# kdavila/lecturemath

Measured on AMD Instinct MI355X. Metric: frames/sec end-to-end binarize+CC+group @1080p, higher is better.
Workload: dtype u8

## Files before the change

lecturemath_amd/csrc/lm_group.hip:

```cpp
#include "lm_stream.h"

#include <sched.h>

#include <algorithm>
#include <atomic>
#include <chrono>
#include <thread>
#include <unordered_map>
#include <vector>

#define LM_SJ_TILE 256

__global__ void __launch_bounds__(256) lm_k_selfjoin(const unsigned long long* __restrict__ box, int n, int* __restrict__ n_pairs,
                                                     int2* __restrict__ pairs, int cap_pairs)
{
    __shared__ unsigned long long s_box[LM_SJ_TILE];
    __shared__ int s_base;
    unsigned mine = 0, off = 0;
    for (int pass = 0; pass < 2; pass++) {
        for (int rt = blockIdx.y * LM_SJ_TILE; rt < n; rt += gridDim.y * LM_SJ_TILE) {
            const int tile = (n - rt < LM_SJ_TILE) ? n - rt : LM_SJ_TILE;
            __syncthreads();
            if ((int)threadIdx.x < tile) s_box[threadIdx.x] = box[rt + threadIdx.x];
            __syncthreads();
// ... 116 lines not shown
{
    const int X0 = it.x0 + un.tx * LM_GT, Y0 = it.y0 + un.ty * LM_GT;
    const int wx0 = r.min_x >> 5, nw = (r.max_x >> 5) - wx0 + 1;
    const int ya = r.min_y > Y0 ? r.min_y : Y0, yb = r.max_y < Y0 + LM_GT - 1 ? r.max_y : Y0 + LM_GT - 1;
    const int ja = (X0 >> 5) > wx0 ? (X0 >> 5) - wx0 : 0;
    const int jb = ((X0 + LM_GT - 1) >> 5) - wx0 < nw - 1 ? ((X0 + LM_GT - 1) >> 5) - wx0 : nw - 1;
    const int tw = jb - ja + 1, total = (tw > 0 && yb >= ya) ? tw * (yb - ya + 1) : 0;
    bool hit = false;
    for (int idx = threadIdx.x; idx < total && !hit; idx += blockDim.x) {
        const int rr = idx / tw, j = ja + (idx - rr * tw);
        unsigned wbits = crop[r.crop_off + (unsigned long long)((ya + rr - r.min_y) * nw + j)];
        const int xw = (wx0 + j) * 32;
        if (xw < X0) wbits &= (X0 - xw >= 32) ? 0u : (0xffffffffu << (X0 - xw));
        if (xw + 31 >= X0 + LM_GT) wbits &= (xw >= X0 + LM_GT) ? 0u : (0xffffffffu >> (xw + 32 - (X0 + LM_GT)));
        hit = wbits != 0u;
    }
    if (hit) *s_hit = 1;
}

LM_DEV void lm_gimg_single_write(const LmGimgItem& it, const LmGimgUnit& un, const LmCcRec& r, const uint32_t* __restrict__ crop, uint32_t* __restrict__ bits)
{
    const int X0 = it.x0 + un.tx * LM_GT, Y0 = it.y0 + un.ty * LM_GT;
    const int wx0 = r.min_x >> 5, nw = (r.max_x >> 5) - wx0 + 1;
    const int tw = (it.w - un.tx * LM_GT < LM_GT) ? it.w - un.tx * LM_GT : LM_GT;
    const int th = (it.h - un.ty * LM_GT < LM_GT) ? it.h - un.ty * LM_GT : LM_GT;
    const int bw = (it.w + 31) >> 5;
    for (int t = threadIdx.x; t < 2 * LM_GT; t += blockDim.x) {
        const int yy = t >> 1, k = t & 1, y = Y0 + yy;
        if (yy >= th || un.tx * 2 + k >= bw || y < r.min_y || y > r.max_y) continue;
        const int xa = X0 + 32 * k;
        const int c0 = (xa >> 5) - wx0, sh = xa & 31;
        const uint32_t* row = crop + r.crop_off + (unsigned long long)(y - r.min_y) * nw;
        const unsigned lo = (c0 >= 0 && c0 < nw) ? row[c0] : 0u;
        const unsigned hi = (sh && c0 + 1 >= 0 && c0 + 1 < nw) ? row[c0 + 1] : 0u;
        unsigned w = sh ? ((lo >> sh) | (hi << (32 - sh))) : lo;
        const int valid = tw - 32 * k;
        if (valid < 32) w &= valid <= 0 ? 0u : ((1u << valid) - 1u);
        if (w) bits[it.bits_off + (long long)(un.ty * LM_GT + yy) * bw + un.tx * 2 + k] = w;
    }
}

LM_DEV int lm_gimg_vmin(int item_max, double thr)
{
    const double mx = (double)item_max;
    int vmin = (int)(thr * mx);
    if (vmin < 0) vmin = 0;
    while (vmin > 0 && (double)(vmin - 1) / mx >= thr) vmin--;
    while ((double)vmin / mx < thr) vmin++;
    return vmin;
}

LM_DEV bool lm_gimg_single_tile(const LmGimgItem& it) { return it.w <= LM_GT && it.h <= LM_GT; }

__global__ void __launch_bounds__(256) lm_k_gimg_max(const LmGimgItem* __restrict__ items, const LmGimgUnit* __restrict__ units,
                                                     const unsigned* __restrict__ n_units_p, const LmGimgMember* __restrict__ members,
                                                     const LmCcRec* __restrict__ cc, const uint32_t* __restrict__ crop,
                                                     int32_t* __restrict__ item_max, double thr, uint32_t* __restrict__ bits)
{
    __shared__ int s_mask[LM_GT * LM_GT];
    __shared__ int s_max;
    const int n_units = (int)*n_units_p;
    for (int u = blockIdx.x; u < n_units; u += gridDim.x) {
        const LmGimgUnit un = units[u];
        const LmGimgItem it = items[un.item];
        if (threadIdx.x == 0) s_max = 0;
        if (un.mem_cnt == 1 && thr > 0.0) {
            const LmGimgMember mem = members[un.mem_off];
            const LmCcRec r = cc[mem.cc];
            __syncthreads();
            lm_gimg_single_hit(it, un, r, crop, &s_max);
            __syncthreads();
            const int tile_max = s_max ? mem.count : 0;
            if (threadIdx.x == 0 && tile_max) atomicMax(&item_max[un.item], tile_max);
            if (lm_gimg_single_tile(it) && tile_max && tile_max >= lm_gimg_vmin(tile_max, thr)) lm_gimg_single_write(it, un, r, crop, bits);
            __syncthreads();
            continue;
        }
        lm_gimg_accumulate(it, un, members, cc, crop, s_mask);
        int mx = 0;
        for (int i = threadIdx.x; i < LM_GT * LM_GT; i += blockDim.x) mx = s_mask[i] > mx ? s_mask[i] : mx;
        if (mx) atomicMax(&s_max, mx);
        __syncthreads();
        const int tile_max = s_max;
        if (threadIdx.x == 0 && tile_max) atomicMax(&item_max[un.item], tile_max);
        if (lm_gimg_single_tile(it) && tile_max) lm_gimg_write_tile(it, un, s_mask, tile_max, thr, bits);
        __syncthreads();
    }
}

__global__ void __launch_bounds__(256) lm_k_gimg_write(const LmGimgItem* __restrict__ items, const LmGimgUnit* __restrict__ units,
                                                       const unsigned* __restrict__ n_units_p, const LmGimgMember* __restrict__ members,
                                                       const LmCcRec* __restrict__ cc, const uint32_t* __restrict__ crop,
                                                       const int32_t* __restrict__ item_max, double thr, uint32_t* __restrict__ bits)
{
    __shared__ int s_mask[LM_GT * LM_GT];
    const int n_units = (int)*n_units_p;
    for (int u = blockIdx.x; u < n_units; u += gridDim.x) {
        const LmGimgUnit un = units[u];
        const LmGimgItem it = items[un.item];
        if (lm_gimg_single_tile(it) && item_max[un.item] > 0) continue;
        if (un.mem_cnt == 1 && thr > 0.0 && item_max[un.item] > 0) {
            const LmGimgMember mem = members[un.mem_off];
            if (mem.count >= lm_gimg_vmin(item_max[un.item], thr)) lm_gimg_single_write(it, un, cc[mem.cc], crop, bits);
            continue;
        }
        lm_gimg_accumulate(it, un, members, cc, crop, s_mask);
        lm_gimg_write_tile(it, un, s_mask, item_max[un.item], thr, bits);
        __syncthreads();
    }
}

struct LmRenderItem { int32_t x0, y0, w, h; long long bits_off; };

#define LM_RT_ROWS 64
#define LM_RT_COLS 256
#define LM_RT_PITCH (LM_RT_COLS / 32 + 1)
#define LM_RT_PLANE (LM_RT_ROWS * LM_RT_PITCH)
#define LM_RT_MAXHIT 96
#define LM_RT_WPL 4

LM_DEV void lm_render_paint(const LmRenderItem& it, int X0, int Y0, const uint32_t* __restrict__ bits, unsigned* s_pl, int lane, int nl)
{
    const int xa = it.x0 > X0 ? it.x0 : X0, xb = (it.x0 + it.w < X0 + LM_RT_COLS) ? it.x0 + it.w : X0 + LM_RT_COLS;
    const int ya = it.y0 > Y0 ? it.y0 : Y0, yb = (it.y0 + it.h < Y0 + LM_RT_ROWS) ? it.y0 + it.h : Y0 + LM_RT_ROWS;
    const int bw = (it.w + 31) >> 5;
    const int jlo = (xa - X0) >> 5, nw = ((xb - 1 - X0) >> 5) - jlo + 1;
    const int total = nw * (yb - ya);
    const float inv = 1.0f / (float)nw;
    const uint32_t* src = bits + it.bits_off + (long long)(ya - it.y0) * bw;
    for (int idx0 = lane; idx0 < total; idx0 += nl * LM_RT_WPL) {
        unsigned lo[LM_RT_WPL], hi[LM_RT_WPL];
        int col[LM_RT_WPL], slot[LM_RT_WPL];
#pragma unroll
        for (int u = 0; u < LM_RT_WPL; u++) {
            const int idx = idx0 + u * nl;
            int yy = (int)((float)idx * inv);
            int j = idx - yy * nw;
            if (j < 0) { yy--; j += nw; }
            if (j >= nw) { yy++; j -= nw; }
            col[u] = X0 + 32 * (jlo + j);
            const int d = col[u] - it.x0;
            const int sw = d >> 5;
            const uint32_t* r = src + (long long)yy * bw;
            const bool on = idx < total;
            lo[u] = (on && sw >= 0 && sw < bw) ? r[sw] : 0u;
            hi[u] = (on && (d & 31) && sw + 1 < bw) ? r[sw + 1] : 0u;
            slot[u] = (ya - Y0 + yy) * LM_RT_PITCH + jlo + j;
        }
#pragma unroll
        for (int u = 0; u < LM_RT_WPL; u++) {
            const int sh = (col[u] - it.x0) & 31;
            unsigned c = sh ? ((lo[u] >> sh) | (hi[u] << (32 - sh))) : lo[u];
            if (col[u] < xa) c &= 0xffffffffu << (xa - col[u]);
            if (col[u] + 32 > xb) c &= 0xffffffffu >> (col[u] + 32 - xb);
            for (int p = 0; p < 8 && c; p++) c &= atomicXor(&s_pl[p * LM_RT_PLANE + slot[u]], c);
        }
    }
}

__global__ void __launch_bounds__(256) lm_k_render_items(const long long* __restrict__ frame_item_off, int F, const int32_t* __restrict__ gpf,
                                                         const int32_t* __restrict__ ages, const int32_t* __restrict__ ages_off,
                                                         const int32_t* __restrict__ bounds, const int64_t* __restrict__ gitem_first,
                                                         const int64_t* __restrict__ gbits_off, LmRenderItem* __restrict__ out)
{
    for (int f = blockIdx.x; f < F; f += gridDim.x)
    for (long long i = frame_item_off[f] + threadIdx.x; i < frame_item_off[f + 1]; i += blockDim.x) {
    const int gi = gpf[i];
    const int32_t* a = ages + ages_off[gi];
    const int na = ages_off[gi + 1] - ages_off[gi];
    LmRenderItem ri;
    ri.x0 = bounds[gi * 4 + 0]; ri.y0 = bounds[gi * 4 + 2];
    ri.w = bounds[gi * 4 + 1] - ri.x0 + 1; ri.h = bounds[gi * 4 + 3] - ri.y0 + 1;
    ri.bits_off = 0;
    if (na < 2) {
        ri.w = 0; ri.h = 0;
    } else {
        int lo = 0, hi = na - 1;
        while (hi - lo > 1) {
            const int mid = (lo + hi) >> 1;
            if (a[mid] < f) lo = mid; else hi = mid;
        }
        const int sidx = lo;
        ri.bits_off = gbits_off[gitem_first[gi] + sidx];
    }
    out[i] = ri;
    }
}

__global__ void __launch_bounds__(256) lm_k_render_frames(const long long* __restrict__ frame_item_off,
                                                          const LmRenderItem* __restrict__ items, const uint32_t* __restrict__ bits,
                                                          int first_frame, int W, int H, uint8_t* __restrict__ out)
{
    __shared__ unsigned s_pl[8 * LM_RT_PLANE];
    __shared__ LmRenderItem s_hit[LM_RT_MAXHIT];
    __shared__ unsigned s_pre[LM_RT_MAXHIT + 1];
    __shared__ int s_nhit;
    const int f = first_frame + blockIdx.z;
    const int X0 = blockIdx.x * LM_RT_COLS, Y0 = blockIdx.y * LM_RT_ROWS;
    for (int i = threadIdx.x; i < 8 * LM_RT_PLANE; i += blockDim.x) s_pl[i] = 0;
    if (threadIdx.x == 0) s_nhit = 0;
    __syncthreads();
    const long long i0 = frame_item_off[f], i1 = frame_item_off[f + 1];
#pragma unroll 2
    for (long long ib = i0 + threadIdx.x; ib < i1; ib += blockDim.x) {
        const LmRenderItem mine = items[ib];
        if (mine.x0 < X0 + LM_RT_COLS && mine.x0 + mine.w > X0 && mine.y0 < Y0 + LM_RT_ROWS && mine.y0 + mine.h > Y0) {
            const int slot = atomicAdd(&s_nhit, 1);
            if (slot < LM_RT_MAXHIT) s_hit[slot] = mine;
            else lm_render_paint(mine, X0, Y0, bits, s_pl, 0, 1);
        }
    }
    __syncthreads();
    const int nhit = s_nhit < LM_RT_MAXHIT ? s_nhit : LM_RT_MAXHIT;
    {
        const int lane = lm_lane();
        if (threadIdx.x < 64) {
            unsigned carry = 0;
            for (int h0 = 0; h0 < nhit; h0 += 64) {
                const int h = h0 + lane;
                unsigned words = 0;
                if (h < nhit) {
                    const LmRenderItem it = s_hit[h];
                    const int xa = it.x0 > X0 ? it.x0 : X0, xb = (it.x0 + it.w < X0 + LM_RT_COLS) ? it.x0 + it.w : X0 + LM_RT_COLS;
                    const int ya = it.y0 > Y0 ? it.y0 : Y0, yb = (it.y0 + it.h < Y0 + LM_RT_ROWS) ? it.y0 + it.h : Y0 + LM_RT_ROWS;
                    const int jlo = (xa - X0) >> 5, nw = ((xb - 1 - X0) >> 5) - jlo + 1;
                    words = (nw > 0 && yb > ya) ? (unsigned)(nw * (yb - ya)) : 0u;
                }
                const unsigned incl = lm_wave_incl_scan(words);
                if (h < nhit) s_pre[h] = carry + incl - words;
                carry += (unsigned)__shfl((int)incl, 63);
            }
            if (lane == 0) s_pre[nhit] = carry;
        }
    }
    __syncthreads();
    {
        const unsigned total = s_pre[nhit];
        for (unsigned g0 = threadIdx.x; g0 < total; g0 += blockDim.x * LM_RT_WPL) {
            unsigned lo[LM_RT_WPL], hi[LM_RT_WPL];
            int col[LM_RT_WPL], slot[LM_RT_WPL], xa_[LM_RT_WPL], xb_[LM_RT_WPL], x0_[LM_RT_WPL];
#pragma unroll
            for (int u = 0; u < LM_RT_WPL; u++) {
                const unsigned g = g0 + (unsigned)u * blockDim.x;
                lo[u] = 0; hi[u] = 0; col[u] = 0; slot[u] = 0; xa_[u] = 0; xb_[u] = 0; x0_[u] = 0;
                if (g < total) {
                    int a = 0, b2 = nhit;
                    while (b2 - a > 1) {
                        const int mid = (a + b2) >> 1;
                        if (s_pre[mid] <= g) a = mid; else b2 = mid;
                    }
                    const LmRenderItem it = s_hit[a];
                    const int xa = it.x0 > X0 ? it.x0 : X0, xb = (it.x0 + it.w < X0 + LM_RT_COLS) ? it.x0 + it.w : X0 + LM_RT_COLS;
                    const int ya = it.y0 > Y0 ? it.y0 : Y0;
                    const int bw = (it.w + 31) >> 5;
                    const int jlo = (xa - X0) >> 5, nw = ((xb - 1 - X0) >> 5) - jlo + 1;
                    const int idx = (int)(g - s_pre[a]);
                    int yy = (int)((float)idx * (1.0f / (float)nw));
                    int j = idx - yy * nw;
                    if (j < 0) { yy--; j += nw; }
                    if (j >= nw) { yy++; j -= nw; }
                    col[u] = X0 + 32 * (jlo + j);
                    const int d = col[u] - it.x0;
                    const int sw = d >> 5;
                    const uint32_t* r = bits + it.bits_off + (long long)(ya - it.y0 + yy) * bw;
                    lo[u] = (sw >= 0 && sw < bw) ? r[sw] : 0u;
                    hi[u] = ((d & 31) && sw + 1 < bw) ? r[sw + 1] : 0u;
                    slot[u] = (ya - Y0 + yy) * LM_RT_PITCH + jlo + j;
                    xa_[u] = xa; xb_[u] = xb; x0_[u] = it.x0;
                }
            }
#pragma unroll
            for (int u = 0; u < LM_RT_WPL; u++) {
                if (g0 + (unsigned)u * blockDim.x >= total) continue;
                const int sh = (col[u] - x0_[u]) & 31;
                unsigned c = sh ? ((lo[u] >> sh) | (hi[u] << (32 - sh))) : lo[u];
                if (col[u] < xa_[u]) c &= 0xffffffffu << (xa_[u] - col[u]);
                if (col[u] + 32 > xb_[u]) c &= 0xffffffffu >> (col[u] + 32 - xb_[u]);
                for (int p = 0; p < 8 && c; p++) c &= atomicXor(&s_pl[p * LM_RT_PLANE + slot[u]], c);
            }
        }
    }
    __syncthreads();
    uint8_t* dst = out + (long long)blockIdx.z * W * H;
    const bool vec = ((W & 15) == 0) && ((((uintptr_t)out) & 15) == 0);
    for (int i = threadIdx.x; i < LM_RT_ROWS * LM_RT_COLS / 16; i += blockDim.x) {
        const int yy = i / (LM_RT_COLS / 16), xq = i - yy * (LM_RT_COLS / 16);
        const int y = Y0 + yy, x = X0 + xq * 16;
        if (y >= H || x >= W) continue;
        unsigned pl[8], upper = 0;
#pragma unroll
        for (int p = 0; p < 8; p++) {
            pl[p] = (s_pl[p * LM_RT_PLANE + yy * LM_RT_PITCH + (xq >> 1)] >> (16 * (xq & 1))) & 0xffffu;
            if (p) upper |= pl[p];
        }
        unsigned o[4];
        if (!upper) {
#pragma unroll
            for (int q = 0; q < 4; q++) o[q] = ((((pl[0] >> (4 * q)) & 15u) * 0x00204081u) & 0x01010101u) * 0xffu;
        } else {
#pragma unroll
            for (int q = 0; q < 4; q++) {
                o[q] = 0;
                for (int t = 0; t < 4; t++) {
                    unsigned k = 0;
                    for (int p = 0; p < 8; p++) k |= ((pl[p] >> (4 * q + t)) & 1u) << p;
                    o[q] |= ((0u - k) & 0xffu) << (8 * t);
                }
            }
        }
        uint8_t* d = dst + (long long)y * W + x;
        if (vec) {
            *(uint4*)d = make_uint4(o[0], o[1], o[2], o[3]);
        } else {
            for (int k = 0; k < 16 && x + k < W; k++) d[k] = (uint8_t)(o[k >> 2] >> (8 * (k & 3)));
        }
    }
}

__global__ void __launch_bounds__(256) lm_k_frame_sums(const uint8_t* __restrict__ frames, long long px, unsigned long long* __restrict__ sums)
{
    const uint8_t* f = frames + (long long)blockIdx.y * px;
    const bool vec = ((((uintptr_t)f) & 15) == 0);
    unsigned long long acc = 0;
    const long long n16 = vec ? (px >> 4) : 0;
    for (long long i = (long long)blockIdx.x * blockDim.x + threadIdx.x; i < n16; i += (long long)gridDim.x * blockDim.x) {
        const uint4 v = *(const uint4*)(f + (i << 4));
        unsigned s4 = 0;
#if LM_HIP_EMULATED
        const unsigned w[4] = {v.x, v.y, v.z, v.w};
        for (int k = 0; k < 4; k++) s4 += (w[k] & 0xffu) + ((w[k] >> 8) & 0xffu) + ((w[k] >> 16) & 0xffu) + (w[k] >> 24);
#else
        s4 = __builtin_amdgcn_sad_u8(v.x, 0u, s4); s4 = __builtin_amdgcn_sad_u8(v.y, 0u, s4);
        s4 = __builtin_amdgcn_sad_u8(v.z, 0u, s4); s4 = __builtin_amdgcn_sad_u8(v.w, 0u, s4);
#endif
        acc += s4;
    }
    for (long long i = (n16 << 4) + (long long)blockIdx.x * blockDim.x + threadIdx.x; i < px; i += (long long)gridDim.x * blockDim.x) acc += f[i];
    __shared__ unsigned long long s_acc;
    if (threadIdx.x == 0) s_acc = 0;
    __syncthreads();
    const unsigned lo = lm_wave_sum((unsigned)(acc & 0xffffffu)), mid = lm_wave_sum((unsigned)((acc >> 24) & 0xffffffu));
    const unsigned hi = lm_wave_sum((unsigned)(acc >> 48));
    if (lm_lane() == 0) atomicAdd(&s_acc, (unsigned long long)lo + ((unsigned long long)mid << 24) + ((unsigned long long)hi << 48));
    __syncthreads();
    if (threadIdx.x == 0 && s_acc) atomicAdd(&sums[blockIdx.y], s_acc);
}

struct LmBitImage { int32_t x0, y0, w, h; long long src_off, bits_off; };

__global__ void __launch_bounds__(256) lm_k_img_pack(const LmBitImage* __restrict__ items, int n, const uint8_t* __restrict__ src,
                                                     uint32_t* __restrict__ bits)
{
    for (int it = blockIdx.y; it < n; it += gridDim.y) {
        const LmBitImage im = items[it];
        const int bw = (im.w + 31) >> 5;
        for (int i = blockIdx.x * blockDim.x + threadIdx.x; i < im.h * bw; i += gridDim.x * blockDim.x) {
            const int y = i / bw, k = i - y * bw;
            const uint8_t* p = src + im.src_off + (long long)y * im.w + k * 32;
            const int lim = (im.w - k * 32 < 32) ? im.w - k * 32 : 32;
            unsigned word = 0;
            for (int b = 0; b < lim; b++) word |= (unsigned)(p[b] != 0) << b;
            bits[im.bits_off + i] = word;
        }
    }
}
// ... 365 lines not shown
{
    for (int k = blockIdx.y; k < n_items; k += gridDim.y) {
        const LmGimgItem it = items[k];
        const int bw = (it.w + 31) >> 5;
        const long long px = (long long)it.w * it.h;
        for (long long i = (long long)blockIdx.x * blockDim.x + threadIdx.x; i < px; i += (long long)gridDim.x * blockDim.x) {
            const int y = (int)(i / it.w), x = (int)(i - (long long)y * it.w);
            images[it.img_off + i] = ((bits[it.bits_off + (long long)y * bw + (x >> 5)] >> (x & 31)) & 1u) ? 255 : 0;
        }
    }
}

struct LmGroups {
    LmStream* s;
    int max_gap, min_times, t_window;
    double min_recall, img_thr;
    int n_frames, n_uniq0;
    int64_t n_split;
    std::vector<int32_t> uniq_cc;
    std::vector<int64_t> ulist_off;
    std::vector<int32_t> ulist_cc;
    std::vector<int32_t> assign;
    std::vector<int32_t> stable;
    int64_t total_intersections;
    std::vector<int64_t> grp_off; std::vector<int32_t> grp_members;
    std::vector<int32_t> gid_of_unique;
    std::vector<int64_t> ages_off; std::vector<int32_t> ages;
    std::vector<int64_t> gpf_off; std::vector<int32_t> gpf;
    std::vector<int32_t> conf_g1, conf_g2; std::vector<int64_t> conf_matched, conf_unmatched, conf_union; std::vector<double> conf_inter;
    std::vector<int32_t> bounds;
    std::vector<int64_t> gimg_off;
    std::vector<int64_t> gimg_item_off;
    bool have_pairs = false, have_nbr = false;
    std::vector<int32_t> pair_a, pair_b, pair_match;
    std::vector<int64_t> tov_off; std::vector<int32_t> tov_other; std::vector<double> tov_recall, tov_precision;
    std::vector<int64_t> aov_off; std::vector<int32_t> aov_other, aov_matched, aov_size_other, aov_size_self;
    std::vector<uint8_t> gimg_host;
    int n_stable = 0;
    long long n_adj = 0, n_aov = 0, n_tov = 0;
    unsigned* d_adj_off = nullptr; int32_t *d_adj = nullptr, *d_arow = nullptr, *d_match = nullptr;
    unsigned *d_aov_off = nullptr, *d_tov_off = nullptr;
    int32_t *d_aov_j = nullptr, *d_aov_other = nullptr, *d_aov_matched = nullptr, *d_aov_size_other = nullptr, *d_aov_size_self = nullptr;
    int32_t* d_tov_other = nullptr; double *d_tov_recall = nullptr, *d_tov_precision = nullptr;
    LmGimgItem* d_items = nullptr;
    int n_items = 0;
    uint32_t* d_gbits = nullptr;
    std::vector<int64_t> gbits_off;
    long long* d_frame_item_off = nullptr;
    LmRenderItem* d_render_items = nullptr;
    std::vector<void*> d_owned;
    char* arena = nullptr;
    size_t arena_cap = 0, arena_used = 0, arena_want = 0;
    bool arena_cached = false;
    char* pin = nullptr;
    size_t pin_cap = 0, pin_used = 0;
    std::vector<void*> pin_owned;
    bool pin_cached = false;
    size_t pin_want = 0;
};

static void* lm_galloc(LmGroups* g, size_t bytes)
{
    const size_t need = (bytes + 255) & ~(size_t)255;
    g->arena_want += need;
    if (g->arena && g->arena_used + need <= g->arena_cap) {
        void* p = g->arena + g->arena_used;
        g->arena_used += need;
        return p;
    }
    void* p = nullptr;
    if (hipMalloc(&p, need ? need : 256) != hipSuccess) { lm_set_error("lm_group_run: hipMalloc(%zu) failed", need); return nullptr; }
    g->d_owned.push_back(p);
    return p;
}

static void* lm_gpin(LmGroups* g, size_t bytes)
{
    const size_t need = (bytes + 255) & ~(size_t)255;
    g->pin_want += need;
    if (g->pin && g->pin_used + need <= g->pin_cap) {
        void* p = g->pin + g->pin_used;
        g->pin_used += need;
        return p;
    }
    void* p = nullptr;
    if (hipHostMalloc(&p, need ? need : 256) != hipSuccess) { lm_set_error("lm_group_run: hipHostMalloc(%zu) failed", need); return nullptr; }
    g->pin_owned.push_back(p);
    return p;
}

#define LM_G_ARRAYS 40
enum {
    LM_G_UNIQ_CC = 0, LM_G_ULIST_OFF, LM_G_ULIST_CC, LM_G_ASSIGN, LM_G_STABLE, LM_G_PAIR_A, LM_G_PAIR_B, LM_G_PAIR_MATCH,
    LM_G_TOV_OFF, LM_G_TOV_OTHER, LM_G_TOV_RECALL, LM_G_TOV_PRECISION, LM_G_AOV_OFF, LM_G_AOV_OTHER, LM_G_AOV_MATCHED,
    LM_G_AOV_SIZE_OTHER, LM_G_AOV_SIZE_SELF, LM_G_GRP_OFF, LM_G_GRP_MEMBERS, LM_G_GID, LM_G_AGES_OFF, LM_G_AGES, LM_G_GPF_OFF,
    LM_G_GPF, LM_G_CONF_G1, LM_G_CONF_G2, LM_G_CONF_MATCHED, LM_G_CONF_UNMATCHED, LM_G_CONF_UNION, LM_G_CONF_INTER, LM_G_BOUNDS,
    LM_G_GIMG_OFF, LM_G_GIMG_ITEM_OFF, LM_G_GIMG, LM_G_SCALARS
};

template <class T> static int lm_upload(LmGroups* g, const std::vector<T>& v, T** d, hipStream_t st)
{
    *d = (T*)lm_galloc(g, (v.size() ? v.size() : 1) * sizeof(T));
    if (!*d) return LM_ERR_HIP;
    if (v.empty()) return LM_OK;
    void* stage = lm_gpin(g, v.size() * sizeof(T));
    if (!stage) return LM_ERR_HIP;
    memcpy(stage, v.data(), v.size() * sizeof(T));
    LM_HIP(hipMemcpyAsync(*d, stage, v.size() * sizeof(T), hipMemcpyHostToDevice, st));
    return LM_OK;
}

template <class T> static int lm_download(LmGroups* g, const T* d, size_t n, std::vector<T>& v, hipStream_t st)
// ... 486 lines not shown
            const unsigned long long b = s_box[(size_t)sidx_of_unique[u]];
            x0 = std::min(x0, (int)(b & 0xffff)); x1 = std::max(x1, (int)((b >> 16) & 0xffff));
            y0 = std::min(y0, (int)((b >> 32) & 0xffff)); y1 = std::max(y1, (int)(b >> 48));
            slot_group[(size_t)i] = gi;
            slot_cc[(size_t)i] = g->uniq_cc[u];
        }
        g->bounds[(size_t)gi * 4 + 0] = x0; g->bounds[(size_t)gi * 4 + 1] = x1; g->bounds[(size_t)gi * 4 + 2] = y0; g->bounds[(size_t)gi * 4 + 3] = y1;
        const int w = x1 - x0 + 1, h = y1 - y0 + 1;
        const int ns = (int)(g->ages_off[(size_t)gi + 1] - g->ages_off[gi]) - 1;
        const long long ntiles = (long long)((w + LM_GT - 1) / LM_GT) * ((h + LM_GT - 1) / LM_GT);
        for (int j = 0; j < ns; j++) {
            LmGimgItem it;
            it.x0 = x0; it.y0 = y0; it.w = w; it.h = h;
            it.img_off = g->gimg_off.back();
            it.bits_off = bit_words;
            g->gbits_off.push_back(bit_words);
            g->gimg_off.push_back(it.img_off + (int64_t)w * h);
            bit_words += (long long)h * ((w + 31) >> 5);
            tile_off.push_back(tile_off.back() + ntiles);
            items.push_back(it);
        }
        g->gimg_item_off.push_back((int64_t)items.size());
    }
    const int n_items = (int)items.size();
    const long long n_tiles = tile_off.back();
    g->n_items = n_items;
    tm.mark("  gimg: items (host)");
    g->d_gbits = (uint32_t*)lm_galloc(g, (size_t)std::max<long long>(bit_words, 1) * sizeof(uint32_t));
    if (!g->d_gbits) return LM_ERR_HIP;
    int64_t* d_gitem_first = nullptr;
    int32_t *d_ages = nullptr;
    if (n_items > 0) {
        LmGimgTab T;
        int32_t *d_slot_group, *d_slot_unique, *d_slot_cc, *d_ulist_frame, *d_bounds_g;
        int64_t *d_ages_off64, *d_ulist_off, *d_tile_off;
        std::vector<int64_t> gitem_first(g->gimg_item_off.begin(), g->gimg_item_off.end() - 1);
        if (lm_upload(g, slot_group, &d_slot_group, st) || lm_upload(g, g->grp_members, &d_slot_unique, st) || lm_upload(g, slot_cc, &d_slot_cc, st) ||
            lm_upload(g, g->ages, &d_ages, st) || lm_upload(g, g->ages_off, &d_ages_off64, st) || lm_upload(g, gitem_first, &d_gitem_first, st) ||
            lm_upload(g, g->ulist_off, &d_ulist_off, st) || lm_upload(g, ulist_frame, &d_ulist_frame, st) || lm_upload(g, tile_off, &d_tile_off, st) ||
            lm_upload(g, items, &g->d_items, st) || lm_upload(g, g->bounds, &d_bounds_g, st))
            return LM_ERR_HIP;
        T.slot_group = d_slot_group; T.slot_unique = d_slot_unique; T.slot_cc = d_slot_cc; T.n_slots = (int)g->grp_members.size();
        T.ages = d_ages; T.ages_off = d_ages_off64; T.gitem_first = d_gitem_first; T.ulist_off = d_ulist_off; T.ulist_frame = d_ulist_frame;
        T.tile_off = d_tile_off; T.bounds = d_bounds_g;
        const size_t nt1 = (size_t)std::max<long long>(n_tiles, 1);
        const int n_chunks = (int)((n_tiles + LM_SCAN_CHUNK - 1) / LM_SCAN_CHUNK);
        unsigned* d_tile_cnt = (unsigned*)lm_galloc(g, (nt1 + 1) * sizeof(unsigned));
        unsigned* d_tile_moff = (unsigned*)lm_galloc(g, (nt1 + 1) * sizeof(unsigned));
        unsigned* d_chunk = (unsigned*)lm_galloc(g, ((size_t)n_chunks + 2) * sizeof(unsigned));
        LmGimgUnit* d_units = (LmGimgUnit*)lm_galloc(g, nt1 * sizeof(LmGimgUnit));
        int32_t* d_max = (int32_t*)lm_galloc(g, (size_t)n_items * sizeof(int32_t));
        unsigned* d_nunits = (unsigned*)lm_galloc(g, 256);
        if (!d_tile_cnt || !d_tile_moff || !d_chunk || !d_units || !d_max || !d_nunits) return LM_ERR_HIP;
        LM_HIP(hipMemsetAsync(d_tile_cnt, 0, (nt1 + 1) * sizeof(unsigned), st));
        LM_HIP(hipMemsetAsync(d_nunits, 0, 256, st));
        LM_HIP(hipMemsetAsync(d_max, 0, (size_t)n_items * sizeof(int32_t), st));
        LM_HIP(hipMemsetAsync(g->d_gbits, 0, (size_t)std::max<long long>(bit_words, 1) * sizeof(uint32_t), st));
        const unsigned sb = lm_gblocks(T.n_slots, 4, 16384);
        hipLaunchKernelGGL((lm_k_gimg_members<0>), dim3(sb), dim3(256), 0, st, T, d_tile_cnt, (const unsigned*)nullptr, (LmGimgMember*)nullptr, s->cc);
        hipLaunchKernelGGL(lm_k_scan_chunks, dim3((unsigned)std::max(n_chunks, 1)), dim3(1024), 0, st, d_tile_cnt, d_tile_moff, n_tiles, d_chunk);
        hipLaunchKernelGGL(lm_k_scan_u32, dim3(1), dim3(1024), 0, st, d_chunk, d_chunk, n_chunks, d_tot + 5);
        hipLaunchKernelGGL(lm_k_scan_add, dim3(lm_gblocks(n_tiles + 1, 256, 4096)), dim3(256), 0, st, d_tile_moff, n_tiles, d_chunk, n_chunks);
        unsigned long long h_nmem = 0;
        LM_HIP(hipMemcpyAsync(&h_nmem, d_tot + 5, sizeof(h_nmem), hipMemcpyDeviceToHost, st));
        LM_HIP(hipStreamSynchronize(st));
        if (h_nmem >= (1ull << 32)) { lm_set_error("lm_group_run: %llu group-image tile members (limit 2^32)", h_nmem); return LM_ERR_CAPACITY; }
        LmGimgMember* d_members = (LmGimgMember*)lm_galloc(g, (size_t)std::max<unsigned long long>(h_nmem, 1) * sizeof(LmGimgMember));
        if (!d_members) return LM_ERR_HIP;
        LM_HIP(hipMemsetAsync(d_tile_cnt, 0, (nt1 + 1) * sizeof(unsigned), st));
        hipLaunchKernelGGL((lm_k_gimg_members<1>), dim3(sb), dim3(256), 0, st, T, d_tile_cnt, d_tile_moff, d_members, s->cc);
        hipLaunchKernelGGL(lm_k_gimg_units, dim3(lm_gblocks(n_tiles, 256, 4096)), dim3(256), 0, st, d_tile_moff, n_tiles, d_tile_off, g->d_items, n_items,
                           g->img_thr > 0.0 ? 0 : 1, d_units, d_nunits);
        tm.mark("  gimg: member + tile tables (device)", st, true);
        const unsigned nb = LM_HIP_EMULATED ? 2u : (unsigned)std::min<long long>(std::max<long long>(n_tiles, 1), 8192);
        hipLaunchKernelGGL(lm_k_gimg_max, dim3(nb), dim3(256), 0, st, g->d_items, d_units, d_nunits, d_members, s->cc, s->crop, d_max, g->img_thr, g->d_gbits);
        hipLaunchKernelGGL(lm_k_gimg_write, dim3(nb), dim3(256), 0, st, g->d_items, d_units, d_nunits, d_members, s->cc, s->crop, d_max, g->img_thr,
                           g->d_gbits);
        LM_HIP(hipGetLastError());
        if (tm.on) {
            unsigned nu_ = 0;
            (void)hipMemcpyAsync(&nu_, d_nunits, 4, hipMemcpyDeviceToHost, st);
            (void)hipStreamSynchronize(st);
            fprintf(stderr, "[lm_group]   groups %d items %d tile members %llu tiles %lld visited %u conflicts %zu\n", nG, n_items, h_nmem, n_tiles, nu_,
                    g->conf_g1.size());
        }
        tm.mark("  gimg: max + write", st, true);
    }
    if (reconstruct_tables) {
        std::vector<long long> fio(g->gpf_off.begin(), g->gpf_off.end());
        std::vector<int32_t> ages_off32(g->ages_off.begin(), g->ages_off.end());
        int32_t *d_gpf, *d_ages_off, *d_bounds;
        int64_t* d_gbits_off;
        const size_t n_ritems = g->gpf.size();
        g->d_render_items = (LmRenderItem*)lm_galloc(g, std::max<size_t>(n_ritems, 1) * sizeof(LmRenderItem));
        if (!g->d_render_items) return LM_ERR_HIP;
        if (lm_upload(g, fio, &g->d_frame_item_off, st)) return LM_ERR_HIP;
        if (n_ritems) {
            if (lm_upload(g, g->gpf, &d_gpf, st) || lm_upload(g, ages_off32, &d_ages_off, st) || lm_upload(g, g->bounds, &d_bounds, st) ||
                lm_upload(g, g->gbits_off, &d_gbits_off, st))
                return LM_ERR_HIP;
            hipLaunchKernelGGL(lm_k_render_items, dim3(lm_gblocks(F, 1, 16384)), dim3(256), 0, st, g->d_frame_item_off, F, d_gpf,
                               d_ages, d_ages_off, d_bounds, d_gitem_first, d_gbits_off, g->d_render_items);
        }
    }
    LM_HIP(hipGetLastError());
    LM_HIP(hipStreamSynchronize(st));
    tm.mark("render tables + final sync");
    return LM_OK;
}

static int lm_group_materialize_pairs(LmGroups* g)
{
    if (g->have_pairs) return LM_OK;
    std::vector<int32_t> adj, arow, match;
    hipStream_t st = nullptr;
    if (g->n_adj > 0 && (lm_download(g, g->d_adj, (size_t)g->n_adj, adj, st) || lm_download(g, g->d_arow, (size_t)g->n_adj, arow, st) ||
                         lm_download(g, g->d_match, (size_t)g->n_adj, match, st)))
        return LM_ERR_HIP;
    g->pair_a.clear(); g->pair_b.clear(); g->pair_match.clear();
    for (long long e = 0; e < g->n_adj; e++)
        if (arow[(size_t)e] < adj[(size_t)e]) {
            g->pair_a.push_back(g->stable[arow[(size_t)e]]); g->pair_b.push_back(g->stable[adj[(size_t)e]]); g->pair_match.push_back(match[(size_t)e]);
        }
    g->have_pairs = true;
    return LM_OK;
}

static int lm_group_materialize_neighbours(LmGroups* g)
{
    if (g->have_nbr) return LM_OK;
    hipStream_t st = nullptr;
    const size_t nU = g->uniq_cc.size();
    const int nS = g->n_stable;
    std::vector<unsigned> aoff, toff;
    g->tov_off.assign(nU + 1, 0); g->aov_off.assign(nU + 1, 0);
    if (nS > 0) {
        if (lm_download(g, g->d_aov_off, (size_t)nS + 1, aoff, st) || lm_download(g, g->d_tov_off, (size_t)nS + 1, toff, st)) return LM_ERR_HIP;
        if (lm_download(g, g->d_aov_other, (size_t)g->n_aov, g->aov_other, st) || lm_download(g, g->d_aov_matched, (size_t)g->n_aov, g->aov_matched, st) ||
            lm_download(g, g->d_aov_size_other, (size_t)g->n_aov, g->aov_size_other, st) ||
            lm_download(g, g->d_aov_size_self, (size_t)g->n_aov, g->aov_size_self, st) || lm_download(g, g->d_tov_other, (size_t)g->n_tov, g->tov_other, st) ||
            lm_download(g, g->d_tov_recall, (size_t)g->n_tov, g->tov_recall, st) || lm_download(g, g->d_tov_precision, (size_t)g->n_tov, g->tov_precision, st))
            return LM_ERR_HIP;
        int si = 0;
        for (size_t u = 0; u < nU; u++) {
            if (si < nS && g->stable[si] == (int32_t)u) {
                g->aov_off[u + 1] = g->aov_off[u] + (int64_t)(aoff[(size_t)si + 1] - aoff[si]);
                g->tov_off[u + 1] = g->tov_off[u] + (int64_t)(toff[(size_t)si + 1] - toff[si]);
                si++;
            } else {
                g->aov_off[u + 1] = g->aov_off[u];
                g->tov_off[u + 1] = g->tov_off[u];
            }
        }
    }
    g->have_nbr = true;
    return LM_OK;
}

extern "C" LmGroups* lm_group_run(LmStream* s, int max_gap, int min_times, int t_window, double min_recall, double img_threshold,
                                  int reconstruct_tables, void* stream)
{
    if (!s) { lm_set_error("lm_group_run: null stream"); return nullptr; }
    LmGroups* g = new LmGroups();
    g->s = s;
    if (!s->garena_busy) {
        if (!s->garena) {
            const LmGeom gm = s->ctx->g;
            size_t first = ((size_t)64 << 20) + (size_t)s->frames_pushed * (size_t)gm.W * (size_t)gm.H / 4;
            if (first > ((size_t)16 << 30)) first = (size_t)16 << 30;
            if (hipMalloc(&s->garena, first) == hipSuccess) s->garena_bytes = first;
            else {
                (void)hipGetLastError();
                first = (size_t)64 << 20;
                if (hipMalloc(&s->garena, first) == hipSuccess) s->garena_bytes = first;
            }
        }
        if (s->garena) { g->arena = (char*)s->garena; g->arena_cap = s->garena_bytes; g->arena_cached = true; s->garena_busy = 1; }
    }
    g->max_gap = max_gap; g->min_times = min_times; g->t_window = t_window;
    g->min_recall = min_recall; g->img_thr = img_threshold;
    if (lm_group_run_impl(g, reconstruct_tables, (hipStream_t)stream) != LM_OK) {
        lm_group_destroy(g);
        return nullptr;
    }
    if (getenv("LM_GROUP_TIMING"))
        fprintf(stderr, "[lm_group] device arena: %zu MB wanted, %zu MB cached; pinned staging: %zu MB wanted, %zu MB cached\n", g->arena_want >> 20,
                g->arena_cap >> 20, g->pin_want >> 20, g->pin_cap >> 20);
    return g;
}

extern "C" int lm_group_render(LmGroups* g, int first, int n, uint8_t* d_out, void* stream)
{
    if (!g || !g->d_frame_item_off || first < 0 || n <= 0 || first + n > g->n_frames || !d_out) {
        lm_set_error("lm_group_render: bad arguments (or lm_group_run was called with reconstruct_tables = 0)");
        return LM_ERR_ARG;
    }
    const LmGeom gm = g->s->ctx->g;
    hipLaunchKernelGGL(lm_k_render_frames, dim3((gm.W + LM_RT_COLS - 1) / LM_RT_COLS, (gm.H + LM_RT_ROWS - 1) / LM_RT_ROWS, n), dim3(256), 0,
                       (hipStream_t)stream, g->d_frame_item_off, g->d_render_items, g->d_gbits, first, gm.W, gm.H, d_out);
    LM_HIP(hipGetLastError());
    return LM_OK;
}

extern "C" int lm_frame_sums(const uint8_t* d_frames, int n_frames, int64_t pixels_per_frame, uint64_t* d_sums, void* stream)
{
    if (!d_frames || !d_sums || n_frames <= 0 || pixels_per_frame <= 0) { lm_set_error("lm_frame_sums: bad arguments"); return LM_ERR_ARG; }
    hipStream_t st = (hipStream_t)stream;
    LM_HIP(hipMemsetAsync(d_sums, 0, (size_t)n_frames * sizeof(uint64_t), st));
    long long bx = (pixels_per_frame / 16 + 255) / 256;
    if (bx > 64) bx = 64;
    if (bx < 1) bx = 1;
    hipLaunchKernelGGL(lm_k_frame_sums, dim3((unsigned)(LM_HIP_EMULATED ? 2 : bx), n_frames), dim3(256), 0, st, d_frames, (long long)pixels_per_frame,
                       (unsigned long long*)d_sums);
    LM_HIP(hipGetLastError());
    return LM_OK;
}

extern "C" int lm_image_pairs_overlap(const int32_t* h_boxes, const uint8_t* h_images, const int64_t* h_img_off, int n, int32_t* h_pairs,
                                      int64_t cap, int64_t* n_pairs, void* stream)
{
    if (!n_pairs || n < 0 || (n > 0 && (!h_boxes || !h_images || !h_img_off)) || cap < 0 || (cap > 0 && !h_pairs)) {
        lm_set_error("lm_image_pairs_overlap: bad arguments");
        return LM_ERR_ARG;
    }
    *n_pairs = 0;
    if (n < 2) return LM_OK;
    hipStream_t st = (hipStream_t)stream;
    std::vector<LmBitImage> items((size_t)n);
    std::vector<unsigned long long> hbox((size_t)n);
    long long words = 0;
    for (int k = 0; k < n; k++) {
        const int32_t* bx = h_boxes + (size_t)k * 4;
        LmBitImage& im = items[(size_t)k];
// ... 114 lines not shown
```

Before: 75200.

## Keep multi-tile gimg accumulated sums in scratch to skip recompute in write pass

For images spanning several tiles, the max pass now compresses each accumulated tile mask to uint8 or uint16 and stores it in a budgeted scratch arena. The write pass then thresholds the stored sums instead of running the member accumulation again. The render kernel also prefetches the first item before clearing shared memory, writes empty tiles with an early-out zero fill, and uses nontemporal vector stores. In exchange it costs extra device memory and scratch traffic, and falls back to recomputing tiles when the budget runs out or the max exceeds 65535.

```diff
diff --git a/lecturemath_amd/csrc/lm_group.hip b/lecturemath_amd/csrc/lm_group.hip
--- a/lecturemath_amd/csrc/lm_group.hip
+++ b/lecturemath_amd/csrc/lm_group.hip
@@ -192,13 +192,113 @@
 
 LM_DEV bool lm_gimg_single_tile(const LmGimgItem& it) { return it.w <= LM_GT && it.h <= LM_GT; }
 
+#define LM_GS_EMPTY 1u
+#define LM_GS_U8 1u
+#define LM_GS_U16 2u
+#define LM_GS_BLOCK 4096u
+struct LmGimgScratch {
+    uint8_t* base;
+    unsigned long long budget;
+    unsigned long long* cursor;
+    uint32_t* unit_store;
+};
+
+typedef unsigned lm_u4v __attribute__((ext_vector_type(4)));
+LM_DEV void lm_gs_put(lm_u4v* p, lm_u4v v)
+{
+#if LM_HIP_EMULATED
+    *p = v;
+#else
+    __builtin_nontemporal_store(v, p);
+#endif
+}
+LM_DEV lm_u4v lm_gs_get(const lm_u4v* p)
+{
+#if LM_HIP_EMULATED
+    return *p;
+#else
+    return __builtin_nontemporal_load(p);
+#endif
+}
+
+LM_DEV void lm_gimg_keep_tile(const int* s_mask, unsigned code, const LmGimgScratch& S)
+{
+    lm_u4v* dst = (lm_u4v*)(S.base + (unsigned long long)((code >> 2) - 1u) * LM_GS_BLOCK);
+    if ((code & 3u) == LM_GS_U8) {
+        const int* m = s_mask + threadIdx.x * 16;
+        lm_u4v v;
+#pragma unroll
+        for (int q = 0; q < 4; q++) v[q] = (unsigned)m[4 * q] | ((unsigned)m[4 * q + 1] << 8) | ((unsigned)m[4 * q + 2] << 16) | ((unsigned)m[4 * q + 3] << 24);
+        lm_gs_put(dst + threadIdx.x, v);
+    } else {
+#pragma unroll
+        for (int k = 0; k < 2; k++) {
+            const int c = k * 256 + (int)threadIdx.x;
+            const int* m = s_mask + c * 8;
+            lm_u4v v;
+#pragma unroll
+            for (int q = 0; q < 4; q++) v[q] = (unsigned)m[2 * q] | ((unsigned)m[2 * q + 1] << 16);
+            lm_gs_put(dst + c, v);
+        }
+    }
+}
+
+LM_DEV void lm_gimg_threshold_kept(const LmGimgItem& it, const LmGimgUnit& un, unsigned code, const LmGimgScratch& S, int vmin,
+                                   uint32_t* __restrict__ bits)
+{
+    const int tw = (it.w - un.tx * LM_GT < LM_GT) ? it.w - un.tx * LM_GT : LM_GT;
+    const int th = (it.h - un.ty * LM_GT < LM_GT) ? it.h - un.ty * LM_GT : LM_GT;
+    const int bw = (it.w + 31) >> 5;
+    const int lane = lm_lane();
+    const lm_u4v* src = (const lm_u4v*)(S.base + (unsigned long long)((code >> 2) - 1u) * LM_GS_BLOCK);
+    const bool u8 = code == LM_GS_EMPTY || (code & 3u) == LM_GS_U8;
+    for (int k = 0; k < (u8 ? 1 : 2); k++) {
+        const int c = k * 256 + (int)threadIdx.x;
+        unsigned m = 0;
+        if (code == LM_GS_EMPTY) {
+            m = vmin <= 0 ? 0xffffu : 0u;
+        } else {
+            const lm_u4v v = lm_gs_get(src + c);
+            if (u8) {
+#pragma unroll
+                for (int q = 0; q < 4; q++)
+#pragma unroll
+                    for (int b = 0; b < 4; b++) m |= ((int)((v[q] >> (8 * b)) & 0xffu) >= vmin ? 1u : 0u) << (4 * q + b);
+            } else {
+#pragma unroll
+                for (int q = 0; q < 4; q++)
+#pragma unroll
+                    for (int b = 0; b < 2; b++) m |= ((int)((v[q] >> (16 * b)) & 0xffffu) >= vmin ? 1u : 0u) << (2 * q + b);
+            }
+        }
+        unsigned w;
+        int yy, kw;
+        if (u8) {
+            w = m << (16 * (lane & 1));
+            w |= (unsigned)__shfl_xor((int)w, 1);
+            yy = c >> 2; kw = (c >> 1) & 1;
+        } else {
+            w = m << (8 * (lane & 3));
+            w |= (unsigned)__shfl_xor((int)w, 1);
+            w |= (unsigned)__shfl_xor((int)w, 2);
+            yy = c >> 3; kw = (c >> 2) & 1;
+        }
+        const int valid = tw - 32 * kw;
+        if (valid < 32) w &= valid <= 0 ? 0u : ((1u << valid) - 1u);
+        const bool writer = u8 ? (lane & 1) == 0 : (lane & 3) == 0;
+        if (writer && yy < th && un.tx * 2 + kw < bw) bits[it.bits_off + (long long)(un.ty * LM_GT + yy) * bw + un.tx * 2 + kw] = w;
+    }
+}
+
 __global__ void __launch_bounds__(256) lm_k_gimg_max(const LmGimgItem* __restrict__ items, const LmGimgUnit* __restrict__ units,
                                                      const unsigned* __restrict__ n_units_p, const LmGimgMember* __restrict__ members,
                                                      const LmCcRec* __restrict__ cc, const uint32_t* __restrict__ crop,
-                                                     int32_t* __restrict__ item_max, double thr, uint32_t* __restrict__ bits)
-{
-    __shared__ int s_mask[LM_GT * LM_GT];
+                                                     int32_t* __restrict__ item_max, double thr, uint32_t* __restrict__ bits,
+                                                     const LmGimgScratch S)
+{
+    __shared__ __attribute__((aligned(16))) int s_mask[LM_GT * LM_GT];
     __shared__ int s_max;
+    __shared__ unsigned s_code;
     const int n_units = (int)*n_units_p;
     for (int u = blockIdx.x; u < n_units; u += gridDim.x) {
         const LmGimgUnit un = units[u];
@@ -223,7 +323,22 @@
         __syncthreads();
         const int tile_max = s_max;
         if (threadIdx.x == 0 && tile_max) atomicMax(&item_max[un.item], tile_max);
-        if (lm_gimg_single_tile(it) && tile_max) lm_gimg_write_tile(it, un, s_mask, tile_max, thr, bits);
+        if (lm_gimg_single_tile(it)) {
+            if (tile_max) lm_gimg_write_tile(it, un, s_mask, tile_max, thr, bits);
+        } else {
+            if (threadIdx.x == 0) {
+                unsigned code = tile_max ? 0u : LM_GS_EMPTY;
+                if (tile_max > 0 && tile_max <= 65535) {
+                    const unsigned long long bytes = tile_max <= 255 ? LM_GS_BLOCK : 2 * LM_GS_BLOCK;
+                    const unsigned long long off = atomicAdd(S.cursor, bytes);
+                    if (off + bytes <= S.budget) code = (((unsigned)(off / LM_GS_BLOCK) + 1u) << 2) | (tile_max <= 255 ? LM_GS_U8 : LM_GS_U16);
+                }
+                S.unit_store[u] = code;
+                s_code = code;
+            }
+            __syncthreads();
+            if (s_code > LM_GS_EMPTY) lm_gimg_keep_tile(s_mask, s_code, S);
+        }
         __syncthreads();
     }
 }
@@ -231,7 +346,8 @@
 __global__ void __launch_bounds__(256) lm_k_gimg_write(const LmGimgItem* __restrict__ items, const LmGimgUnit* __restrict__ units,
                                                        const unsigned* __restrict__ n_units_p, const LmGimgMember* __restrict__ members,
                                                        const LmCcRec* __restrict__ cc, const uint32_t* __restrict__ crop,
-                                                       const int32_t* __restrict__ item_max, double thr, uint32_t* __restrict__ bits)
+                                                       const int32_t* __restrict__ item_max, double thr, uint32_t* __restrict__ bits,
+                                                       const LmGimgScratch S)
 {
     __shared__ int s_mask[LM_GT * LM_GT];
     const int n_units = (int)*n_units_p;
@@ -244,9 +360,28 @@
             if (mem.count >= lm_gimg_vmin(item_max[un.item], thr)) lm_gimg_single_write(it, un, cc[mem.cc], crop, bits);
             continue;
         }
+        const unsigned code = S.unit_store[u];
+        if (code) {
+            lm_gimg_threshold_kept(it, un, code, S, lm_gimg_vmin(item_max[un.item], thr), bits);
+            continue;
+        }
         lm_gimg_accumulate(it, un, members, cc, crop, s_mask);
         lm_gimg_write_tile(it, un, s_mask, item_max[un.item], thr, bits);
         __syncthreads();
+    }
+}
+
+__global__ void __launch_bounds__(256) lm_k_gimg_store_stats(const LmGimgItem* __restrict__ items, const LmGimgUnit* __restrict__ units,
+                                                             const unsigned* __restrict__ n_units_p, const int32_t* __restrict__ item_max,
+                                                             double thr, const uint32_t* __restrict__ unit_store, unsigned* __restrict__ out)
+{
+    const int n_units = (int)*n_units_p;
+    for (int u = (int)(blockIdx.x * blockDim.x + threadIdx.x); u < n_units; u += (int)(gridDim.x * blockDim.x)) {
+        const LmGimgUnit un = units[u];
+        const bool has_max = item_max[un.item] > 0;
+        if ((lm_gimg_single_tile(items[un.item]) && has_max) || (un.mem_cnt == 1 && thr > 0.0 && has_max)) continue;
+        const unsigned code = unit_store[u];
+        atomicAdd(&out[code == 0 ? 3 : (code == LM_GS_EMPTY ? 2 : ((code & 3u) == LM_GS_U8 ? 0 : 1))], 1u);
     }
 }
 
@@ -337,13 +472,15 @@
     __shared__ int s_nhit;
     const int f = first_frame + blockIdx.z;
     const int X0 = blockIdx.x * LM_RT_COLS, Y0 = blockIdx.y * LM_RT_ROWS;
+    const long long i0 = frame_item_off[f], i1 = frame_item_off[f + 1];
+    LmRenderItem first_item = {0, 0, 0, 0, 0};
+    if (i0 + threadIdx.x < i1) first_item = items[i0 + threadIdx.x];
     for (int i = threadIdx.x; i < 8 * LM_RT_PLANE; i += blockDim.x) s_pl[i] = 0;
     if (threadIdx.x == 0) s_nhit = 0;
     __syncthreads();
-    const long long i0 = frame_item_off[f], i1 = frame_item_off[f + 1];
 #pragma unroll 2
     for (long long ib = i0 + threadIdx.x; ib < i1; ib += blockDim.x) {
-        const LmRenderItem mine = items[ib];
+        const LmRenderItem mine = ib == i0 + threadIdx.x ? first_item : items[ib];
         if (mine.x0 < X0 + LM_RT_COLS && mine.x0 + mine.w > X0 && mine.y0 < Y0 + LM_RT_ROWS && mine.y0 + mine.h > Y0) {
             const int slot = atomicAdd(&s_nhit, 1);
             if (slot < LM_RT_MAXHIT) s_hit[slot] = mine;
@@ -351,6 +488,16 @@
         }
     }
     __syncthreads();
+    uint8_t* dst = out + (long long)blockIdx.z * W * H;
+    const bool vec = ((W & 15) == 0) && ((((uintptr_t)out) & 15) == 0);
+    if (s_nhit == 0 && vec) {
+        for (int i = threadIdx.x; i < LM_RT_ROWS * LM_RT_COLS / 16; i += blockDim.x) {
+            const int yy = i / (LM_RT_COLS / 16), xq = i - yy * (LM_RT_COLS / 16);
+            const int y = Y0 + yy, x = X0 + xq * 16;
+            if (y < H && x < W) lm_gs_put((lm_u4v*)(dst + (long long)y * W + x), (lm_u4v)(0u));
+        }
+        return;
+    }
     const int nhit = s_nhit < LM_RT_MAXHIT ? s_nhit : LM_RT_MAXHIT;
     {
         const int lane = lm_lane();
@@ -421,8 +568,6 @@
         }
     }
     __syncthreads();
-    uint8_t* dst = out + (long long)blockIdx.z * W * H;
-    const bool vec = ((W & 15) == 0) && ((((uintptr_t)out) & 15) == 0);
     for (int i = threadIdx.x; i < LM_RT_ROWS * LM_RT_COLS / 16; i += blockDim.x) {
         const int yy = i / (LM_RT_COLS / 16), xq = i - yy * (LM_RT_COLS / 16);
         const int y = Y0 + yy, x = X0 + xq * 16;
@@ -450,7 +595,9 @@
         }
         uint8_t* d = dst + (long long)y * W + x;
         if (vec) {
-            *(uint4*)d = make_uint4(o[0], o[1], o[2], o[3]);
+            lm_u4v v;
+            v[0] = o[0]; v[1] = o[1]; v[2] = o[2]; v[3] = o[3];
+            lm_gs_put((lm_u4v*)d, v);
         } else {
             for (int k = 0; k < 16 && x + k < W; k++) d[k] = (uint8_t)(o[k >> 2] >> (8 * (k & 3)));
         }
@@ -922,12 +1069,20 @@
     char* arena = nullptr;
     size_t arena_cap = 0, arena_used = 0, arena_want = 0;
     bool arena_cached = false;
+    size_t gimg_scratch_budget = 0;
     char* pin = nullptr;
     size_t pin_cap = 0, pin_used = 0;
     std::vector<void*> pin_owned;
     bool pin_cached = false;
     size_t pin_want = 0;
 };
+
+static size_t lm_arena_first_guess(const LmStream* s)
+{
+    const LmGeom gm = s->ctx->g;
+    const size_t first = ((size_t)64 << 20) + (size_t)s->frames_pushed * (size_t)gm.W * (size_t)gm.H / 4;
+    return std::min(first, (size_t)16 << 30);
+}
 
 static void* lm_galloc(LmGroups* g, size_t bytes)
 {
@@ -1520,6 +1675,14 @@
         int32_t* d_max = (int32_t*)lm_galloc(g, (size_t)n_items * sizeof(int32_t));
         unsigned* d_nunits = (unsigned*)lm_galloc(g, 256);
         if (!d_tile_cnt || !d_tile_moff || !d_chunk || !d_units || !d_max || !d_nunits) return LM_ERR_HIP;
+        LmGimgScratch S;
+        S.budget = std::min<unsigned long long>(g->gimg_scratch_budget, (unsigned long long)nt1 * 2 * LM_GS_BLOCK) / LM_GS_BLOCK * LM_GS_BLOCK;
+        S.base = S.budget ? (uint8_t*)lm_galloc(g, (size_t)S.budget + LM_GS_BLOCK) : nullptr;
+        S.cursor = (unsigned long long*)(d_nunits + 2);
+        S.unit_store = (uint32_t*)lm_galloc(g, nt1 * sizeof(uint32_t));
+        if ((S.budget && !S.base) || !S.unit_store) return LM_ERR_HIP;
+        if (S.base) S.base += (LM_GS_BLOCK - ((uintptr_t)S.base & (LM_GS_BLOCK - 1))) & (LM_GS_BLOCK - 1);
+        LM_HIP(hipMemsetAsync(S.unit_store, 0, nt1 * sizeof(uint32_t), st));
         LM_HIP(hipMemsetAsync(d_tile_cnt, 0, (nt1 + 1) * sizeof(unsigned), st));
         LM_HIP(hipMemsetAsync(d_nunits, 0, 256, st));
         LM_HIP(hipMemsetAsync(d_max, 0, (size_t)n_items * sizeof(int32_t), st));
@@ -1541,18 +1704,30 @@
                            g->img_thr > 0.0 ? 0 : 1, d_units, d_nunits);
         tm.mark("  gimg: member + tile tables (device)", st, true);
         const unsigned nb = LM_HIP_EMULATED ? 2u : (unsigned)std::min<long long>(std::max<long long>(n_tiles, 1), 8192);
-        hipLaunchKernelGGL(lm_k_gimg_max, dim3(nb), dim3(256), 0, st, g->d_items, d_units, d_nunits, d_members, s->cc, s->crop, d_max, g->img_thr, g->d_gbits);
+        hipLaunchKernelGGL(lm_k_gimg_max, dim3(nb), dim3(256), 0, st, g->d_items, d_units, d_nunits, d_members, s->cc, s->crop, d_max, g->img_thr, g->d_gbits,
+                           S);
+        LM_HIP(hipGetLastError());
+        tm.mark("  gimg: max + keep sums", st, true);
         hipLaunchKernelGGL(lm_k_gimg_write, dim3(nb), dim3(256), 0, st, g->d_items, d_units, d_nunits, d_members, s->cc, s->crop, d_max, g->img_thr,
-                           g->d_gbits);
+                           g->d_gbits, S);
         LM_HIP(hipGetLastError());
+        tm.mark("  gimg: write (threshold kept sums)", st, true);
         if (tm.on) {
-            unsigned nu_ = 0;
+            unsigned nu_ = 0, h_st[4] = {0, 0, 0, 0};
+            unsigned long long h_asked = 0;
+            unsigned* d_st = d_nunits + 8;
+            hipLaunchKernelGGL(lm_k_gimg_store_stats, dim3(lm_gblocks(n_tiles, 256, 1024)), dim3(256), 0, st, g->d_items, d_units, d_nunits, d_max,
+                               g->img_thr, S.unit_store, d_st);
             (void)hipMemcpyAsync(&nu_, d_nunits, 4, hipMemcpyDeviceToHost, st);
+            (void)hipMemcpyAsync(h_st, d_st, sizeof(h_st), hipMemcpyDeviceToHost, st);
+            (void)hipMemcpyAsync(&h_asked, S.cursor, sizeof(h_asked), hipMemcpyDeviceToHost, st);
             (void)hipStreamSynchronize(st);
             fprintf(stderr, "[lm_group]   groups %d items %d tile members %llu tiles %lld visited %u conflicts %zu\n", nG, n_items, h_nmem, n_tiles, nu_,
                     g->conf_g1.size());
-        }
-        tm.mark("  gimg: max + write", st, true);
+            fprintf(stderr, "[lm_group]   gimg sums: kept %u (uint8 %u, uint16 %u) empty %u recomputed %u; scratch asked %llu bytes, budget %llu bytes\n",
+                    h_st[0] + h_st[1], h_st[0], h_st[1], h_st[2], h_st[3], h_asked, (unsigned long long)S.budget);
+        }
+        tm.mark("  gimg: counters", st, true);
     }
     if (reconstruct_tables) {
         std::vector<long long> fio(g->gpf_off.begin(), g->gpf_off.end());
@@ -1633,9 +1808,7 @@
     g->s = s;
     if (!s->garena_busy) {
         if (!s->garena) {
-            const LmGeom gm = s->ctx->g;
-            size_t first = ((size_t)64 << 20) + (size_t)s->frames_pushed * (size_t)gm.W * (size_t)gm.H / 4;
-            if (first > ((size_t)16 << 30)) first = (size_t)16 << 30;
+            size_t first = lm_arena_first_guess(s);
             if (hipMalloc(&s->garena, first) == hipSuccess) s->garena_bytes = first;
             else {
                 (void)hipGetLastError();
@@ -1647,6 +1820,10 @@
     }
     g->max_gap = max_gap; g->min_times = min_times; g->t_window = t_window;
     g->min_recall = min_recall; g->img_thr = img_threshold;
+    {
+        static const long long forced = [] { const char* e = getenv("LM_GIMG_SCRATCH_BYTES"); return e ? atoll(e) : -1ll; }();
+        g->gimg_scratch_budget = forced >= 0 ? (size_t)forced : lm_arena_first_guess(s) / 4;
+    }
     if (lm_group_run_impl(g, reconstruct_tables, (hipStream_t)stream) != LM_OK) {
         lm_group_destroy(g);
         return nullptr;
```

Measured after the change: 68530. 0.911x the previous value.
